# Antiparadox/Spartan-BN254

Measured on AMD Instinct MI355X. Metric: msm_points_per_s, higher is better.
Workload: dtype u32; 1 GPU; synthetic BN254 G1 MSM, 2^20 uniform Fr scalars x distinct bases per GPU, inputs resident in HBM; steps_in_flight=6

## Files before the change

spartan-bn254_amd/csrc/sort2_kernels.cuh:

```cuda
#pragma once
#include "msm_kernels.cuh"
#include <utility>

namespace sbn {

struct S2Geom {
  size_t n;
  int c, W, P;
  int lo_log;
  int K;
  size_t half, gap;
};

template <int C, int SW = 8> struct S2Shape {
  static constexpr int BITS = SW == 8 ? 254 : 127;
  static constexpr int W0 = (BITS + C - 1) / C;
  static constexpr int W = W0 + ((BITS - (W0 - 1) * C) > C - 1 ? 1 : 0);
};
typedef uint32_t s2_u32x8 __attribute__((ext_vector_type(8)));
template <int C, int w> __device__ __forceinline__ int s2_digit(const s2_u32x8 k, uint32_t& carry) {
  constexpr int bit = w * C, limb = bit >> 5, sh = bit & 31;
  uint64_t x = 0;
  if constexpr (limb < 8) x = k[limb];
  if constexpr (limb + 1 < 8) x |= (uint64_t)k[limb + 1] << 32;
  const uint32_t raw = (uint32_t)(x >> sh) & ((1u << C) - 1u);
  const uint32_t v = raw + carry;
  if (v >= (1u << (C - 1))) { carry = 1; return (int)v - (1 << C); }
  carry = 0;
  return (int)v;
}
template <int SW = 8> __device__ __forceinline__ s2_u32x8 s2_load_scalar(const uint32_t* __restrict__ scalars, size_t t) {
  const uint4* p = reinterpret_cast<const uint4*>(scalars + (size_t)SW * t);
  const uint4 a = p[0], b = SW == 8 ? p[1] : make_uint4(0u, 0u, 0u, 0u);
  s2_u32x8 k; k[0] = a.x; k[1] = a.y; k[2] = a.z; k[3] = a.w; k[4] = b.x; k[5] = b.y; k[6] = b.z; k[7] = b.w;
  return k;
}
__device__ __forceinline__ bool s2_is_canonical(const s2_u32x8 k) { uint32_t kk[8]; for (int i = 0; i < 8; i++) kk[i] = k[i]; return fe_is_canonical<FrP>(kk); }

extern __shared__ uint32_t s2_lds[];

template <int C, int... Ws>
__device__ __forceinline__ void s2_count_scalar(const s2_u32x8 kk, int P, int lo_log, std::integer_sequence<int, Ws...>) {
  uint32_t carry = 0;
  auto one = [&](auto wc) {
    constexpr int w = decltype(wc)::value;
    const int d = s2_digit<C, w>(kk, carry);
    if (d != 0) atomicAdd(&s2_lds[w * P + (((d < 0 ? -d : d) - 1) >> lo_log)], 1u);
  };
  (one(std::integral_constant<int, Ws>{}), ...);
}
template <int C, int SPT, int SW = 8>
__global__ void __launch_bounds__(1024) k_s2_count(const uint32_t* __restrict__ scalars, S2Geom g, uint32_t* __restrict__ cntA, uint32_t* __restrict__ bad) {
  constexpr int W = S2Shape<C, SW>::W; constexpr int CH = 1024 * SPT;
  const int k = blockIdx.x, P = g.P;
  for (int j = threadIdx.x; j < W * P; j += 1024) s2_lds[j] = 0;
  __syncthreads();
  for (int i = 0; i < SPT; i++) {
    const size_t t = (size_t)k * CH + (size_t)i * 1024 + threadIdx.x;
    if (t >= g.n) break;
    const s2_u32x8 kk = s2_load_scalar<SW>(scalars, t);
    if (SW == 8 && !s2_is_canonical(kk)) atomicAdd(bad, 1u);
    s2_count_scalar<C>(kk, P, g.lo_log, std::make_integer_sequence<int, W>{});
  }
  __syncthreads();
  for (int j = threadIdx.x; j < W * P; j += 1024) cntA[(size_t)j * g.K + k] = s2_lds[j];
}

__device__ __forceinline__ uint32_t s2_block_scan(uint32_t v, uint32_t* tmp , uint32_t* total) {
  const int lane = threadIdx.x & 63, wv = threadIdx.x >> 6, nw = (blockDim.x + 63) >> 6;
  uint32_t inc = v;
#pragma unroll
  for (int d = 1; d < 64; d <<= 1) { const uint32_t o = __shfl_up(inc, d); if (lane >= d) inc += o; }
  if (lane == 63) tmp[wv] = inc;
  __syncthreads();
  if (threadIdx.x == 0) { uint32_t run = 0; for (int i = 0; i < nw; i++) { const uint32_t x = tmp[i]; tmp[i] = run; run += x; } tmp[16] = run; }
  __syncthreads();
  const uint32_t r = inc - v + tmp[wv];
  *total = tmp[16];
  __syncthreads();
  return r;
}
__global__ void __launch_bounds__(256) k_s2_prefix_k(uint32_t* __restrict__ cntA, int K, uint32_t* __restrict__ part_cnt) {
  __shared__ uint32_t tmp[17];
  uint32_t* row = cntA + (size_t)blockIdx.x * K;
  const int per = (K + 255) / 256, b0 = threadIdx.x * per;
  uint32_t sum = 0;
  for (int i = 0; i < per; i++) if (b0 + i < K) sum += row[b0 + i];
  uint32_t total; uint32_t run = s2_block_scan(sum, tmp, &total);
  for (int i = 0; i < per; i++) if (b0 + i < K) { const uint32_t v = row[b0 + i]; row[b0 + i] = run; run += v; }
  if (threadIdx.x == 0) part_cnt[blockIdx.x] = total;
}
__global__ void __launch_bounds__(1024) k_s2_prefix_hi(const uint32_t* __restrict__ part_cnt, int W, int P, uint32_t* __restrict__ part_off, uint32_t* __restrict__ sc_off) {
  __shared__ uint32_t tmp[17];
  __shared__ uint32_t wstart[32];
  const int n = W * P, per = (n + 1023) / 1024, i0 = (int)threadIdx.x * per, i1 = (i0 + per < n) ? i0 + per : n;
  uint32_t sv = 0, sk = 0;
  for (int i = i0; i < i1; i++) { const uint32_t v = part_cnt[i]; sv += v; sk += (v + S2_SUB - 1) / S2_SUB; }
  uint32_t tv, tk;
  uint32_t rv = s2_block_scan(sv, tmp, &tv), rk = s2_block_scan(sk, tmp, &tk);
  for (int i = i0; i < i1; i++) { const uint32_t v = part_cnt[i]; part_off[i] = rv; sc_off[i] = rk; rv += v; rk += (v + S2_SUB - 1) / S2_SUB; }
  if (threadIdx.x == 0) sc_off[(size_t)n] = tk;
  __syncthreads();
  if ((int)threadIdx.x < W) wstart[threadIdx.x] = part_off[(size_t)threadIdx.x * P];
  __syncthreads();
  for (int i = i0; i < i1; i++) part_off[i] -= wstart[i / P];
}

__host__ __device__ inline size_t s2_scatter_lds_bytes(int P, int spt = S2_SPT) { return ((size_t)3 * P + 32) * 4 + (size_t)1024 * spt * 8; }
struct S2ScatterArgs {
  const uint32_t* cntA; const uint32_t* part_off; uint32_t* tmp_idx; uint16_t* tmp_lo;
  size_t n, half, gap; int P, K, k, lo_log;
};
template <int C, int w, int SPT>
__device__ __forceinline__ void s2_scatter_window(const s2_u32x8 (&kk)[SPT], uint32_t (&carry)[SPT], const S2ScatterArgs& a) {
  constexpr int CH = 1024 * SPT;
  const int P = a.P, tid = threadIdx.x;
  uint32_t* cnt = s2_lds; uint32_t* base = cnt + P; uint32_t* gdelta = base + P; uint32_t* tmp = gdelta + P;
  uint32_t* stage_idx = tmp + 32;
  uint16_t* stage_lo = reinterpret_cast<uint16_t*>(stage_idx + CH); uint16_t* stage_hi = stage_lo + CH;
  for (int j = tid; j < P; j += 1024) cnt[j] = 0;
  __syncthreads();
  int d[SPT]; uint32_t rank[SPT];
#pragma unroll
  for (int i = 0; i < SPT; i++) {
    const int dd = s2_digit<C, w>(kk[i], carry[i]);
    d[i] = dd; rank[i] = 0;
    if (dd != 0) rank[i] = atomicAdd(&cnt[((dd < 0 ? -dd : dd) - 1) >> a.lo_log], 1u);
  }
  __syncthreads();
  uint32_t total;
  {
    const uint32_t v = tid < P ? cnt[tid] : 0;
    const uint32_t r = s2_block_scan(v, tmp, &total);
    if (tid < P) { base[tid] = r; gdelta[tid] = a.part_off[(size_t)w * P + tid] + a.cntA[((size_t)w * P + tid) * a.K + a.k] - r; }
  }
  __syncthreads();
  const size_t t0 = (size_t)a.k * CH + tid;
#pragma unroll
  for (int i = 0; i < SPT; i++) {
    if (d[i] == 0) continue;
    const uint32_t b = (uint32_t)((d[i] < 0 ? -d[i] : d[i]) - 1), hi = b >> a.lo_log;
    const uint32_t pos = base[hi] + rank[i];
    size_t e = t0 + (size_t)i * 1024;
    if (a.gap && e >= a.half) e += a.gap;
    stage_idx[pos] = (uint32_t)e | (d[i] < 0 ? 0x80000000u : 0u);
    stage_lo[pos] = (uint16_t)(b & ((1u << a.lo_log) - 1u)); stage_hi[pos] = (uint16_t)hi;
  }
  __syncthreads();
  uint32_t* oi = a.tmp_idx + (size_t)w * a.n; uint16_t* ol = a.tmp_lo + (size_t)w * a.n;
  for (uint32_t j = tid; j < total; j += 1024) {
    const uint32_t pos = j + gdelta[stage_hi[j]];
    oi[pos] = stage_idx[j]; ol[pos] = stage_lo[j];
  }
  __syncthreads();
}
template <int C, int SPT, int... Ws>
__device__ __forceinline__ void s2_scatter_windows(const s2_u32x8 (&kk)[SPT], uint32_t (&carry)[SPT], const S2ScatterArgs& a, std::integer_sequence<int, Ws...>) {
  (s2_scatter_window<C, Ws, SPT>(kk, carry, a), ...);
}
template <int C, int SPT, int SW = 8>
__global__ void __launch_bounds__(1024) k_s2_scatter(const uint32_t* __restrict__ scalars, S2Geom g, const uint32_t* __restrict__ cntA ,
                                                     const uint32_t* __restrict__ part_off, uint32_t* __restrict__ tmp_idx, uint16_t* __restrict__ tmp_lo) {
  S2ScatterArgs a; a.cntA = cntA; a.part_off = part_off; a.tmp_idx = tmp_idx; a.tmp_lo = tmp_lo; a.n = g.n; a.P = g.P; a.K = g.K; a.k = blockIdx.x; a.lo_log = g.lo_log;
  a.half = g.half; a.gap = SW == 8 ? 0 : g.gap;
  s2_u32x8 kk[SPT]; uint32_t carry[SPT];
#pragma unroll
  for (int i = 0; i < SPT; i++) {
    const size_t t = (size_t)blockIdx.x * (1024 * SPT) + (size_t)i * 1024 + threadIdx.x;
    carry[i] = 0;
    kk[i] = t < g.n ? s2_load_scalar<SW>(scalars, t) : (s2_u32x8)(0u);
  }
  s2_scatter_windows<C, SPT>(kk, carry, a, std::make_integer_sequence<int, S2Shape<C, SW>::W>{});
}

__device__ __forceinline__ bool s2_decode(const S2Geom& g, const uint32_t* __restrict__ sc_off, int& q, uint32_t& sidx, uint32_t& k2) {
  const uint32_t Lid = blockIdx.x, xcd = Lid & 7u, slot = Lid >> 3;
  sidx = (slot >> 4) * 128u + xcd * 16u + (slot & 15u);
  const int WP = g.W * g.P;
  if (sidx >= sc_off[WP]) return false;
  int lo = 0, hi = WP;
  while (hi - lo > 1) { const int mid = (lo + hi) >> 1; if (sc_off[mid] <= sidx) lo = mid; else hi = mid; }
  q = lo; k2 = sidx - sc_off[q];
  return true;
}
__host__ __device__ inline uint32_t s2_level2_blocks(size_t max_subchunks) { return (uint32_t)(((max_subchunks + 127) / 128) * 128); }
__device__ __forceinline__ void s2_range(const S2Geom& g, const uint32_t* __restrict__ part_off, const uint32_t* __restrict__ part_cnt, int q, uint32_t k2, size_t& e0, size_t& e1) {
  const uint32_t start = part_off[q], cn = part_cnt[q];
  uint32_t a = k2 * S2_SUB, b = a + S2_SUB; if (a > cn) a = cn; if (b > cn) b = cn;
  const size_t w = (size_t)(q / g.P);
  e0 = w * g.n + start + a; e1 = w * g.n + start + b;
}
__global__ void __launch_bounds__(1024) k_s2_hist(const uint16_t* __restrict__ tmp_lo, S2Geom g, const uint32_t* __restrict__ part_off, const uint32_t* __restrict__ part_cnt, const uint32_t* __restrict__ sc_off, uint32_t* __restrict__ blockhist) {
  __shared__ uint32_t h[S2_LO_MAX];
  int q; uint32_t sidx, k2; if (!s2_decode(g, sc_off, q, sidx, k2)) return;
  const int LO = 1 << g.lo_log;
  for (int j = threadIdx.x; j < LO; j += 1024) h[j] = 0;
  __syncthreads();
  size_t e0, e1; s2_range(g, part_off, part_cnt, q, k2, e0, e1);
  for (size_t e = e0 + threadIdx.x; e < e1; e += 1024) atomicAdd(&h[tmp_lo[e]], 1u);
  __syncthreads();
  uint32_t* o = blockhist + (size_t)sidx * LO;
  for (int j = threadIdx.x; j < LO; j += 1024) o[j] = h[j];
}
__global__ void __launch_bounds__(1024) k_s2_prefix2(uint32_t* __restrict__ blockhist, S2Geom g, const uint32_t* __restrict__ part_off, const uint32_t* __restrict__ sc_off, uint32_t* __restrict__ hist, uint32_t* __restrict__ offs) {
  __shared__ uint32_t tmp[17];
  const int q = blockIdx.x, LO = 1 << g.lo_log, w = q / g.P, hi = q - w * g.P;
  const uint32_t s0 = sc_off[q], nk = sc_off[q + 1] - s0;
  const int j0 = 2 * threadIdx.x;
  uint32_t r0 = 0, r1 = 0;
  if (j0 < LO) {
    uint2* col = reinterpret_cast<uint2*>(blockhist + (size_t)s0 * LO + j0);
    for (uint32_t k = 0; k < nk; k++) { uint2* pq = col + (size_t)k * (LO / 2); const uint2 v = *pq; *pq = make_uint2(r0, r1); r0 += v.x; r1 += v.y; }
  }
  uint32_t total; const uint32_t r = s2_block_scan(r0 + r1, tmp, &total);
  if (j0 < LO) {
    const size_t b = ((size_t)w * g.P + hi) * LO + j0;
    hist[b] = r0; hist[b + 1] = r1;
    offs[b] = part_off[q] + r; offs[b + 1] = part_off[q] + r + r0;
  }
}
constexpr int S2_EPT = 8;
__host__ __device__ inline size_t s2_place_lds_bytes(int lo_log) { return ((size_t)3 * ((size_t)1 << lo_log) + 32) * 4 + (size_t)1024 * S2_EPT * 6; }
__global__ void __launch_bounds__(1024) k_s2_place(const uint16_t* __restrict__ tmp_lo, const uint32_t* __restrict__ tmp_idx, S2Geom g, const uint32_t* __restrict__ part_off, const uint32_t* __restrict__ part_cnt,
                                                   const uint32_t* __restrict__ sc_off, const uint32_t* __restrict__ blockhist ,
                                                   const uint32_t* __restrict__ offs, uint32_t* __restrict__ sorted, size_t estride) {
  constexpr uint32_t T = 1024 * S2_EPT;
  int q; uint32_t sidx, k2; if (!s2_decode(g, sc_off, q, sidx, k2)) return;
  const int LO = 1 << g.lo_log, tid = threadIdx.x;
  uint32_t* cnt = s2_lds; uint32_t* base = cnt + LO; uint32_t* cur = base + LO; uint32_t* tmp = cur + LO;
  uint32_t* stage_idx = tmp + 32; uint16_t* stage_lo = reinterpret_cast<uint16_t*>(stage_idx + T);
  const int w = q / g.P, hi = q - w * g.P;
  const size_t nb = (size_t)g.P << g.lo_log;
  const uint32_t* b0 = blockhist + (size_t)sidx * LO;
  const uint32_t* of = offs + (size_t)w * nb + ((size_t)hi << g.lo_log);
  for (int j = tid; j < LO; j += 1024) { cur[j] = of[j] + b0[j]; cnt[j] = 0; }
  __syncthreads();
  size_t e0, e1; s2_range(g, part_off, part_cnt, q, k2, e0, e1);
  uint32_t* out = sorted + (size_t)w * estride;
  for (size_t tile = e0; tile < e1; tile += T) {
    uint32_t lo[S2_EPT], idx[S2_EPT], rank[S2_EPT];
#pragma unroll
    for (int i = 0; i < S2_EPT; i++) {
      const size_t e = tile + (size_t)i * 1024 + tid;
      lo[i] = 0xffffffffu;
      if (e < e1) { lo[i] = tmp_lo[e]; idx[i] = tmp_idx[e]; rank[i] = atomicAdd(&cnt[lo[i]], 1u); }
    }
    __syncthreads();
    uint32_t total;
    {
      const int j0 = 2 * tid, j1 = 2 * tid + 1;
      const uint32_t v0 = j0 < LO ? cnt[j0] : 0, v1 = j1 < LO ? cnt[j1] : 0;
      const uint32_t r = s2_block_scan(v0 + v1, tmp, &total);
      if (j0 < LO) base[j0] = r;
      if (j1 < LO) base[j1] = r + v0;
    }
    __syncthreads();
#pragma unroll
    for (int i = 0; i < S2_EPT; i++) {
      if (lo[i] == 0xffffffffu) continue;
      const uint32_t pos = base[lo[i]] + rank[i];
      stage_idx[pos] = idx[i]; stage_lo[pos] = (uint16_t)lo[i];
    }
    __syncthreads();
    for (uint32_t j = tid; j < total; j += 1024) {
      const uint32_t l = stage_lo[j];
      out[cur[l] + (j - base[l])] = stage_idx[j];
    }
    __syncthreads();
    for (int j = tid; j < LO; j += 1024) { cur[j] += cnt[j]; cnt[j] = 0; }
    __syncthreads();
  }
}

}
```

spartan-bn254_amd/csrc/glv_kernels.cuh:

```cuda
#pragma once
#include "msm_kernels.cuh"

namespace sbn {

namespace glv {
constexpr uint64_t A[2] = {0x8211bbeb7d4f1128ull, 0x6f4d8248eeb859fcull};
constexpr uint64_t B = 0x89d3256894d213e3ull;
constexpr uint64_t C[2] = {0x0be4e1541221250bull, 0x6f4d8248eeb859fdull};
constexpr uint64_t G1[3] = {0x5398fd0300ff6565ull, 0x4ccef014a773d2d2ull, 0x2ull};
constexpr uint64_t G2[2] = {0xd91d232ec7e0b3d7ull, 0x2ull};
constexpr uint64_t R[4] = {0x43e1f593f0000001ull, 0x2833e84879b97091ull, 0xb85045b68181585dull, 0x30644e72e131a029ull};
constexpr uint32_t BETA[8] = {0x607cfd48u, 0xe4bd44e5u, 0xbb966e3du, 0xc28f069fu, 0xe0acccb0u, 0x5e6dd9e7u, 0xe131a029u, 0x30644e72u};
}

template <int NA, int NB>
__device__ __forceinline__ void glv_mul(const uint64_t (&a)[NA], const uint64_t (&b)[NB], uint64_t (&out)[NA + NB]) {
#pragma unroll
  for (int i = 0; i < NA + NB; i++) out[i] = 0;
#pragma unroll
  for (int i = 0; i < NA; i++) {
    uint64_t carry = 0;
#pragma unroll
    for (int j = 0; j < NB; j++) {
      const uint64_t lo = a[i] * b[j], hi = __umul64hi(a[i], b[j]);
      uint64_t s = out[i + j] + lo; uint64_t cy = s < lo ? 1 : 0;
      s += carry; cy += s < carry ? 1 : 0;
      out[i + j] = s; carry = hi + cy;
    }
    out[i + NB] = carry;
  }
}
template <int NB>
__device__ __forceinline__ void glv_mul_lo256(const uint64_t (&a)[4], const uint64_t (&b)[NB], uint64_t (&out)[4]) {
#pragma unroll
  for (int i = 0; i < 4; i++) out[i] = 0;
#pragma unroll
  for (int i = 0; i < 4; i++) {
    uint64_t carry = 0;
#pragma unroll
    for (int j = 0; j < NB && i + j < 4; j++) {
      const uint64_t lo = a[i] * b[j], hi = __umul64hi(a[i], b[j]);
      uint64_t s = out[i + j] + lo; uint64_t cy = s < lo ? 1 : 0;
      s += carry; cy += s < carry ? 1 : 0;
      out[i + j] = s; carry = hi + cy;
    }
    if (i + NB < 4) out[i + NB] = carry;
  }
}
__device__ __forceinline__ bool glv_diff_ge_r(const uint64_t (&x)[4], const uint64_t (&y)[4]) {
  uint64_t d[4], borrow = 0;
#pragma unroll
  for (int i = 0; i < 4; i++) { const uint64_t t = x[i] - y[i]; const uint64_t b1 = x[i] < y[i]; d[i] = t - borrow; borrow = b1 | (t < borrow); }
#pragma unroll
  for (int i = 3; i >= 0; i--) { if (d[i] != glv::R[i]) return d[i] > glv::R[i]; }
  return true;
}
__device__ __forceinline__ void u128_mul_lo(uint64_t a0, uint64_t a1, uint64_t b0, uint64_t b1, uint64_t& o0, uint64_t& o1) {
  o0 = a0 * b0; o1 = __umul64hi(a0, b0) + a0 * b1 + a1 * b0;
}
__device__ __forceinline__ void u128_add(uint64_t& x0, uint64_t& x1, uint64_t y0, uint64_t y1) { const uint64_t s = x0 + y0; x1 += y1 + (s < x0 ? 1 : 0); x0 = s; }
__device__ __forceinline__ void u128_sub(uint64_t& x0, uint64_t& x1, uint64_t y0, uint64_t y1) { const uint64_t b = x0 < y0 ? 1 : 0; x0 -= y0; x1 -= y1 + b; }

__device__ __forceinline__ void glv_split(const uint64_t (&k)[4], uint64_t (&k1)[2], uint64_t (&k2)[2]) {
  uint64_t p1[7], p2[6];
  glv_mul<4, 3>(k, glv::G1, p1);
  glv_mul<4, 2>(k, glv::G2, p2);
  uint64_t c1[2] = {p1[4], p1[5]}, c2[1] = {p2[4]};
  {
    uint64_t kc[4], cr[4];
    glv_mul_lo256<2>(k, glv::C, kc);
    const uint64_t c1v[4] = {c1[0], c1[1], 0, 0};
    glv_mul_lo256<4>(c1v, glv::R, cr);
    if (glv_diff_ge_r(kc, cr)) { if (++c1[0] == 0) ++c1[1]; }
  }
  {
    uint64_t kb[4], cr[4];
    const uint64_t bb[1] = {glv::B};
    glv_mul_lo256<1>(k, bb, kb);
    const uint64_t c2v[4] = {c2[0], 0, 0, 0};
    glv_mul_lo256<4>(c2v, glv::R, cr);
    if (glv_diff_ge_r(kb, cr)) ++c2[0];
  }
  uint64_t x0 = k[0], x1 = k[1], t0, t1;
  u128_mul_lo(c1[0], c1[1], glv::A[0], glv::A[1], t0, t1); u128_sub(x0, x1, t0, t1);
  u128_mul_lo(c2[0], 0, glv::B, 0, t0, t1); u128_sub(x0, x1, t0, t1);
  uint64_t y0, y1;
  u128_mul_lo(c1[0], c1[1], glv::B, 0, y0, y1);
  u128_mul_lo(c2[0], 0, glv::C[0], glv::C[1], t0, t1); u128_sub(y0, y1, t0, t1);
  if (y1 >> 63) { u128_add(x0, x1, glv::B, 0); u128_add(y0, y1, glv::C[0], glv::C[1]); }
  k1[0] = x0; k1[1] = x1; k2[0] = y0; k2[1] = y1;
}

__global__ void __launch_bounds__(256) k_glv_split(const uint32_t* __restrict__ scalars, size_t n, uint32_t* __restrict__ out, uint32_t* __restrict__ bad) {
  const size_t t = (size_t)blockIdx.x * blockDim.x + threadIdx.x;
  if (t >= n) return;
  const uint4 a = reinterpret_cast<const uint4*>(scalars + 8 * t)[0], b = reinterpret_cast<const uint4*>(scalars + 8 * t)[1];
  const uint32_t kk[8] = {a.x, a.y, a.z, a.w, b.x, b.y, b.z, b.w};
  uint64_t k1[2] = {0, 0}, k2[2] = {0, 0};
  if (!fe_is_canonical<FrP>(kk)) atomicAdd(bad, 1u);
  else {
    const uint64_t k[4] = {(uint64_t)a.x | ((uint64_t)a.y << 32), (uint64_t)a.z | ((uint64_t)a.w << 32), (uint64_t)b.x | ((uint64_t)b.y << 32), (uint64_t)b.z | ((uint64_t)b.w << 32)};
    glv_split(k, k1, k2);
  }
  uint4* o = reinterpret_cast<uint4*>(out);
  o[t] = make_uint4((uint32_t)k1[0], (uint32_t)(k1[0] >> 32), (uint32_t)k1[1], (uint32_t)(k1[1] >> 32));
  o[n + t] = make_uint4((uint32_t)k2[0], (uint32_t)(k2[0] >> 32), (uint32_t)k2[1], (uint32_t)(k2[1] >> 32));
}

__global__ void __launch_bounds__(256) k_glv_table(const uint32_t* __restrict__ pts, size_t npts, uint32_t* __restrict__ out) {
  const size_t j = (size_t)blockIdx.x * blockDim.x + threadIdx.x;
  if (j >= npts) return;
  const uint4* s = reinterpret_cast<const uint4*>(pts + 16 * j);
  uint4* d0 = reinterpret_cast<uint4*>(out + 16 * j);
  uint4* d1 = reinterpret_cast<uint4*>(out + 16 * (npts + j));
  const uint4 w0 = s[0], w1 = s[1], w2 = s[2], w3 = s[3];
  d0[0] = w0; d0[1] = w1; d0[2] = w2; d0[3] = w3;
  const Fq beta = fe_to_mont(fe_unpack<FqP>(glv::BETA));
  const Fq x = fe_load<FqP>(pts + 16 * j);
  fe_store<FqP>(out + 16 * (npts + j), fe_mul(x, beta));
  d1[2] = w2; d1[3] = w3;
}

}
```

Before: 788.2 million points/s.

## Cut barriers and prefetch in MSM sort scatter, hist and place kernels

The scatter kernel now double-buffers its per-window counters, packs the staging entries into uint2, prefetches the next window's global offset and drops several __syncthreads. Sub-chunk decode becomes a parallel search that also caches part_off and part_cnt in shared memory. The hist kernel reads tmp_lo eight entries at a time with uint4 loads. The place kernel loads both tiles of a sub-chunk up front, takes a fast path for sub-chunks of at most 1024 elements, and sets a launch-bounds occupancy hint. These changes target barrier and load-latency overhead in the bucket sort, at the cost of extra registers and tighter assumptions such as S2_SUB equal to two tiles.

```diff
diff --git a/spartan-bn254_amd/csrc/sort2_kernels.cuh b/spartan-bn254_amd/csrc/sort2_kernels.cuh
--- a/spartan-bn254_amd/csrc/sort2_kernels.cuh
+++ b/spartan-bn254_amd/csrc/sort2_kernels.cuh
@@ -66,7 +66,7 @@
   for (int j = threadIdx.x; j < W * P; j += 1024) cntA[(size_t)j * g.K + k] = s2_lds[j];
 }
 
-__device__ __forceinline__ uint32_t s2_block_scan(uint32_t v, uint32_t* tmp , uint32_t* total) {
+__device__ __forceinline__ uint32_t s2_block_scan_open(uint32_t v, uint32_t* tmp , uint32_t* total) {
   const int lane = threadIdx.x & 63, wv = threadIdx.x >> 6, nw = (blockDim.x + 63) >> 6;
   uint32_t inc = v;
 #pragma unroll
@@ -77,6 +77,10 @@
   __syncthreads();
   const uint32_t r = inc - v + tmp[wv];
   *total = tmp[16];
+  return r;
+}
+__device__ __forceinline__ uint32_t s2_block_scan(uint32_t v, uint32_t* tmp , uint32_t* total) {
+  const uint32_t r = s2_block_scan_open(v, tmp, total);
   __syncthreads();
   return r;
 }
@@ -111,15 +115,19 @@
   const uint32_t* cntA; const uint32_t* part_off; uint32_t* tmp_idx; uint16_t* tmp_lo;
   size_t n, half, gap; int P, K, k, lo_log;
 };
-template <int C, int w, int SPT>
-__device__ __forceinline__ void s2_scatter_window(const s2_u32x8 (&kk)[SPT], uint32_t (&carry)[SPT], const S2ScatterArgs& a) {
+__device__ __forceinline__ uint32_t s2_scatter_goff(const S2ScatterArgs& a, int w) {
+  const size_t j = (size_t)w * a.P + threadIdx.x;
+  return (int)threadIdx.x < a.P ? a.part_off[j] + a.cntA[j * a.K + a.k] : 0u;
+}
+template <int C, int w, int W, int SPT>
+__device__ __forceinline__ void s2_scatter_window(const s2_u32x8 (&kk)[SPT], uint32_t (&carry)[SPT], const S2ScatterArgs& a, uint32_t& gpre) {
   constexpr int CH = 1024 * SPT;
   const int P = a.P, tid = threadIdx.x;
-  uint32_t* cnt = s2_lds; uint32_t* base = cnt + P; uint32_t* gdelta = base + P; uint32_t* tmp = gdelta + P;
-  uint32_t* stage_idx = tmp + 32;
-  uint16_t* stage_lo = reinterpret_cast<uint16_t*>(stage_idx + CH); uint16_t* stage_hi = stage_lo + CH;
-  for (int j = tid; j < P; j += 1024) cnt[j] = 0;
-  __syncthreads();
+  uint2* stage = reinterpret_cast<uint2*>(s2_lds);
+  uint32_t* ctr = s2_lds + 2 * CH; uint32_t* gdelta = ctr + 2 * P; uint32_t* tmp = gdelta + P;
+  uint32_t* cnt = ctr + (w & 1) * P; uint32_t* other = ctr + ((w + 1) & 1) * P;
+  uint32_t gnext = 0;
+  if constexpr (w + 1 < W) gnext = s2_scatter_goff(a, w + 1);
   int d[SPT]; uint32_t rank[SPT];
 #pragma unroll
   for (int i = 0; i < SPT; i++) {
@@ -131,8 +139,9 @@
   uint32_t total;
   {
     const uint32_t v = tid < P ? cnt[tid] : 0;
-    const uint32_t r = s2_block_scan(v, tmp, &total);
-    if (tid < P) { base[tid] = r; gdelta[tid] = a.part_off[(size_t)w * P + tid] + a.cntA[((size_t)w * P + tid) * a.K + a.k] - r; }
+    if (tid < P) other[tid] = 0;
+    const uint32_t r = s2_block_scan_open(v, tmp, &total);
+    if (tid < P) { cnt[tid] = r; gdelta[tid] = gpre - r; }
   }
   __syncthreads();
   const size_t t0 = (size_t)a.k * CH + tid;
@@ -140,23 +149,23 @@
   for (int i = 0; i < SPT; i++) {
     if (d[i] == 0) continue;
     const uint32_t b = (uint32_t)((d[i] < 0 ? -d[i] : d[i]) - 1), hi = b >> a.lo_log;
-    const uint32_t pos = base[hi] + rank[i];
+    const uint32_t pos = cnt[hi] + rank[i];
     size_t e = t0 + (size_t)i * 1024;
     if (a.gap && e >= a.half) e += a.gap;
-    stage_idx[pos] = (uint32_t)e | (d[i] < 0 ? 0x80000000u : 0u);
-    stage_lo[pos] = (uint16_t)(b & ((1u << a.lo_log) - 1u)); stage_hi[pos] = (uint16_t)hi;
+    stage[pos] = make_uint2((uint32_t)e | (d[i] < 0 ? 0x80000000u : 0u), (b & ((1u << a.lo_log) - 1u)) | (hi << 16));
   }
   __syncthreads();
   uint32_t* oi = a.tmp_idx + (size_t)w * a.n; uint16_t* ol = a.tmp_lo + (size_t)w * a.n;
   for (uint32_t j = tid; j < total; j += 1024) {
-    const uint32_t pos = j + gdelta[stage_hi[j]];
-    oi[pos] = stage_idx[j]; ol[pos] = stage_lo[j];
-  }
-  __syncthreads();
+    const uint2 s = stage[j];
+    const uint32_t pos = j + gdelta[s.y >> 16];
+    oi[pos] = s.x; ol[pos] = (uint16_t)s.y;
+  }
+  gpre = gnext;
 }
 template <int C, int SPT, int... Ws>
-__device__ __forceinline__ void s2_scatter_windows(const s2_u32x8 (&kk)[SPT], uint32_t (&carry)[SPT], const S2ScatterArgs& a, std::integer_sequence<int, Ws...>) {
-  (s2_scatter_window<C, Ws, SPT>(kk, carry, a), ...);
+__device__ __forceinline__ void s2_scatter_windows(const s2_u32x8 (&kk)[SPT], uint32_t (&carry)[SPT], const S2ScatterArgs& a, uint32_t& gpre, std::integer_sequence<int, Ws...>) {
+  (s2_scatter_window<C, Ws, (int)sizeof...(Ws), SPT>(kk, carry, a, gpre), ...);
 }
 template <int C, int SPT, int SW = 8>
 __global__ void __launch_bounds__(1024) k_s2_scatter(const uint32_t* __restrict__ scalars, S2Geom g, const uint32_t* __restrict__ cntA ,
@@ -164,42 +173,62 @@
   S2ScatterArgs a; a.cntA = cntA; a.part_off = part_off; a.tmp_idx = tmp_idx; a.tmp_lo = tmp_lo; a.n = g.n; a.P = g.P; a.K = g.K; a.k = blockIdx.x; a.lo_log = g.lo_log;
   a.half = g.half; a.gap = SW == 8 ? 0 : g.gap;
   s2_u32x8 kk[SPT]; uint32_t carry[SPT];
+  uint32_t gpre = s2_scatter_goff(a, 0);
 #pragma unroll
   for (int i = 0; i < SPT; i++) {
     const size_t t = (size_t)blockIdx.x * (1024 * SPT) + (size_t)i * 1024 + threadIdx.x;
     carry[i] = 0;
     kk[i] = t < g.n ? s2_load_scalar<SW>(scalars, t) : (s2_u32x8)(0u);
   }
-  s2_scatter_windows<C, SPT>(kk, carry, a, std::make_integer_sequence<int, S2Shape<C, SW>::W>{});
-}
-
-__device__ __forceinline__ bool s2_decode(const S2Geom& g, const uint32_t* __restrict__ sc_off, int& q, uint32_t& sidx, uint32_t& k2) {
-  const uint32_t Lid = blockIdx.x, xcd = Lid & 7u, slot = Lid >> 3;
-  sidx = (slot >> 4) * 128u + xcd * 16u + (slot & 15u);
+  for (int j = threadIdx.x; j < 2 * g.P; j += 1024) s2_lds[2 * (1024 * SPT) + j] = 0;
+  __syncthreads();
+  s2_scatter_windows<C, SPT>(kk, carry, a, gpre, std::make_integer_sequence<int, S2Shape<C, SW>::W>{});
+}
+
+struct S2Sub { int q; uint32_t sidx, k2, start, cn; };
+__device__ __forceinline__ bool s2_decode(const S2Geom& g, const uint32_t* __restrict__ sc_off, const uint32_t* __restrict__ part_off, const uint32_t* __restrict__ part_cnt, uint32_t* sh, S2Sub& s) {
+  const uint32_t Lid = blockIdx.x, xcd = Lid & 7u, slot = Lid >> 3, sidx = (slot >> 4) * 128u + xcd * 16u + (slot & 15u);
   const int WP = g.W * g.P;
-  if (sidx >= sc_off[WP]) return false;
-  int lo = 0, hi = WP;
-  while (hi - lo > 1) { const int mid = (lo + hi) >> 1; if (sc_off[mid] <= sidx) lo = mid; else hi = mid; }
-  q = lo; k2 = sidx - sc_off[q];
+  const uint32_t nsc = sc_off[WP];
+  for (int j = threadIdx.x; j < WP; j += blockDim.x) {
+    const uint32_t a = sc_off[j], b = sc_off[j + 1];
+    if (a <= sidx && sidx < b) { sh[0] = (uint32_t)j; sh[1] = sidx - a; sh[2] = part_off[j]; sh[3] = part_cnt[j]; }
+  }
+  if (sidx >= nsc) return false;
+  __syncthreads();
+  s.sidx = sidx; s.q = (int)sh[0]; s.k2 = sh[1]; s.start = sh[2]; s.cn = sh[3];
   return true;
 }
 __host__ __device__ inline uint32_t s2_level2_blocks(size_t max_subchunks) { return (uint32_t)(((max_subchunks + 127) / 128) * 128); }
-__device__ __forceinline__ void s2_range(const S2Geom& g, const uint32_t* __restrict__ part_off, const uint32_t* __restrict__ part_cnt, int q, uint32_t k2, size_t& e0, size_t& e1) {
-  const uint32_t start = part_off[q], cn = part_cnt[q];
-  uint32_t a = k2 * S2_SUB, b = a + S2_SUB; if (a > cn) a = cn; if (b > cn) b = cn;
-  const size_t w = (size_t)(q / g.P);
-  e0 = w * g.n + start + a; e1 = w * g.n + start + b;
+__device__ __forceinline__ void s2_range(const S2Geom& g, const S2Sub& s, size_t& e0, size_t& e1) {
+  uint32_t a = s.k2 * S2_SUB, b = a + S2_SUB; if (a > s.cn) a = s.cn; if (b > s.cn) b = s.cn;
+  const size_t w = (size_t)(s.q / g.P);
+  e0 = w * g.n + s.start + a; e1 = w * g.n + s.start + b;
 }
 __global__ void __launch_bounds__(1024) k_s2_hist(const uint16_t* __restrict__ tmp_lo, S2Geom g, const uint32_t* __restrict__ part_off, const uint32_t* __restrict__ part_cnt, const uint32_t* __restrict__ sc_off, uint32_t* __restrict__ blockhist) {
   __shared__ uint32_t h[S2_LO_MAX];
-  int q; uint32_t sidx, k2; if (!s2_decode(g, sc_off, q, sidx, k2)) return;
+  __shared__ uint32_t dec[4];
   const int LO = 1 << g.lo_log;
   for (int j = threadIdx.x; j < LO; j += 1024) h[j] = 0;
-  __syncthreads();
-  size_t e0, e1; s2_range(g, part_off, part_cnt, q, k2, e0, e1);
-  for (size_t e = e0 + threadIdx.x; e < e1; e += 1024) atomicAdd(&h[tmp_lo[e]], 1u);
-  __syncthreads();
-  uint32_t* o = blockhist + (size_t)sidx * LO;
+  S2Sub s; if (!s2_decode(g, sc_off, part_off, part_cnt, dec, s)) return;
+  size_t e0, e1; s2_range(g, s, e0, e1);
+  const size_t a0 = ((e0 + 7) & ~(size_t)7) < e1 ? ((e0 + 7) & ~(size_t)7) : e1, a1 = a0 + ((e1 - a0) & ~(size_t)7);
+  if (e0 + threadIdx.x < a0) atomicAdd(&h[tmp_lo[e0 + threadIdx.x]], 1u);
+  if (a1 + threadIdx.x < e1) atomicAdd(&h[tmp_lo[a1 + threadIdx.x]], 1u);
+  const uint4* v = reinterpret_cast<const uint4*>(tmp_lo + a0);
+  const uint32_t ng = (uint32_t)((a1 - a0) >> 3);
+  auto add8 = [&](const uint4 x) {
+    atomicAdd(&h[x.x & 0xffffu], 1u); atomicAdd(&h[x.x >> 16], 1u); atomicAdd(&h[x.y & 0xffffu], 1u); atomicAdd(&h[x.y >> 16], 1u);
+    atomicAdd(&h[x.z & 0xffffu], 1u); atomicAdd(&h[x.z >> 16], 1u); atomicAdd(&h[x.w & 0xffffu], 1u); atomicAdd(&h[x.w >> 16], 1u);
+  };
+  for (uint32_t i = threadIdx.x; i < ng; i += 2048) {
+    const bool two = i + 1024 < ng;
+    const uint4 x = v[i], y = two ? v[i + 1024] : make_uint4(0u, 0u, 0u, 0u);
+    add8(x);
+    if (two) add8(y);
+  }
+  __syncthreads();
+  uint32_t* o = blockhist + (size_t)s.sidx * LO;
   for (int j = threadIdx.x; j < LO; j += 1024) o[j] = h[j];
 }
 __global__ void __launch_bounds__(1024) k_s2_prefix2(uint32_t* __restrict__ blockhist, S2Geom g, const uint32_t* __restrict__ part_off, const uint32_t* __restrict__ sc_off, uint32_t* __restrict__ hist, uint32_t* __restrict__ offs) {
@@ -221,51 +250,80 @@
 }
 constexpr int S2_EPT = 8;
 __host__ __device__ inline size_t s2_place_lds_bytes(int lo_log) { return ((size_t)3 * ((size_t)1 << lo_log) + 32) * 4 + (size_t)1024 * S2_EPT * 6; }
-__global__ void __launch_bounds__(1024) k_s2_place(const uint16_t* __restrict__ tmp_lo, const uint32_t* __restrict__ tmp_idx, S2Geom g, const uint32_t* __restrict__ part_off, const uint32_t* __restrict__ part_cnt,
+__global__ void __launch_bounds__(1024, 8) k_s2_place(const uint16_t* __restrict__ tmp_lo, const uint32_t* __restrict__ tmp_idx, S2Geom g, const uint32_t* __restrict__ part_off, const uint32_t* __restrict__ part_cnt,
                                                    const uint32_t* __restrict__ sc_off, const uint32_t* __restrict__ blockhist ,
                                                    const uint32_t* __restrict__ offs, uint32_t* __restrict__ sorted, size_t estride) {
   constexpr uint32_t T = 1024 * S2_EPT;
-  int q; uint32_t sidx, k2; if (!s2_decode(g, sc_off, q, sidx, k2)) return;
+  static_assert(S2_SUB == 2 * T, "a sub-chunk is two tiles: both are loaded before the first is sorted");
   const int LO = 1 << g.lo_log, tid = threadIdx.x;
   uint32_t* cnt = s2_lds; uint32_t* base = cnt + LO; uint32_t* cur = base + LO; uint32_t* tmp = cur + LO;
   uint32_t* stage_idx = tmp + 32; uint16_t* stage_lo = reinterpret_cast<uint16_t*>(stage_idx + T);
-  const int w = q / g.P, hi = q - w * g.P;
+  S2Sub s; if (!s2_decode(g, sc_off, part_off, part_cnt, tmp + 20, s)) return;
+  const int w = s.q / g.P, hi = s.q - w * g.P;
   const size_t nb = (size_t)g.P << g.lo_log;
-  const uint32_t* b0 = blockhist + (size_t)sidx * LO;
+  const uint32_t* b0 = blockhist + (size_t)s.sidx * LO;
   const uint32_t* of = offs + (size_t)w * nb + ((size_t)hi << g.lo_log);
-  for (int j = tid; j < LO; j += 1024) { cur[j] = of[j] + b0[j]; cnt[j] = 0; }
-  __syncthreads();
-  size_t e0, e1; s2_range(g, part_off, part_cnt, q, k2, e0, e1);
+  size_t e0, e1; s2_range(g, s, e0, e1);
   uint32_t* out = sorted + (size_t)w * estride;
-  for (size_t tile = e0; tile < e1; tile += T) {
-    uint32_t lo[S2_EPT], idx[S2_EPT], rank[S2_EPT];
+  const uint32_t m = (uint32_t)(e1 - e0);
+  if (m <= 1024) {
+    uint32_t l = 0, ix = 0, dst = 0;
+    const bool have = (uint32_t)tid < m;
+    if (have) { l = tmp_lo[e0 + tid]; ix = tmp_idx[e0 + tid]; dst = of[l] + b0[l]; cnt[l] = 0; }
+    __syncthreads();
+    if (have) out[dst + atomicAdd(&cnt[l], 1u)] = ix;
+    return;
+  }
+  uint32_t c0[2];
+#pragma unroll
+  for (int i = 0; i < 2; i++) { const int j = tid + 1024 * i; c0[i] = j < LO ? of[j] + b0[j] : 0u; }
+  uint32_t lo[2][S2_EPT], idx[2][S2_EPT];
+#pragma unroll
+  for (int t = 0; t < 2; t++) {
 #pragma unroll
     for (int i = 0; i < S2_EPT; i++) {
-      const size_t e = tile + (size_t)i * 1024 + tid;
-      lo[i] = 0xffffffffu;
-      if (e < e1) { lo[i] = tmp_lo[e]; idx[i] = tmp_idx[e]; rank[i] = atomicAdd(&cnt[lo[i]], 1u); }
+      const size_t e = e0 + (size_t)t * T + (size_t)i * 1024 + tid;
+      lo[t][i] = e < e1 ? (uint32_t)tmp_lo[e] : 0xffffffffu;
+    }
+#pragma unroll
+    for (int i = 0; i < S2_EPT; i++) {
+      const size_t e = e0 + (size_t)t * T + (size_t)i * 1024 + tid;
+      idx[t][i] = e < e1 ? tmp_idx[e] : 0u;
+    }
+  }
+#pragma unroll
+  for (int i = 0; i < 2; i++) { const int j = tid + 1024 * i; if (j < LO) { cur[j] = c0[i]; cnt[j] = 0; } }
+  __syncthreads();
+#pragma unroll
+  for (int t = 0; t < 2; t++) {
+    uint32_t rank[S2_EPT];
+#pragma unroll
+    for (int i = 0; i < S2_EPT; i++) {
+      rank[i] = 0;
+      if (lo[t][i] != 0xffffffffu) rank[i] = atomicAdd(&cnt[lo[t][i]], 1u);
     }
     __syncthreads();
     uint32_t total;
     {
       const int j0 = 2 * tid, j1 = 2 * tid + 1;
       const uint32_t v0 = j0 < LO ? cnt[j0] : 0, v1 = j1 < LO ? cnt[j1] : 0;
-      const uint32_t r = s2_block_scan(v0 + v1, tmp, &total);
+      const uint32_t r = s2_block_scan_open(v0 + v1, tmp, &total);
       if (j0 < LO) base[j0] = r;
       if (j1 < LO) base[j1] = r + v0;
     }
     __syncthreads();
 #pragma unroll
     for (int i = 0; i < S2_EPT; i++) {
-      if (lo[i] == 0xffffffffu) continue;
-      const uint32_t pos = base[lo[i]] + rank[i];
-      stage_idx[pos] = idx[i]; stage_lo[pos] = (uint16_t)lo[i];
+      if (lo[t][i] == 0xffffffffu) continue;
+      const uint32_t pos = base[lo[t][i]] + rank[i];
+      stage_idx[pos] = idx[t][i]; stage_lo[pos] = (uint16_t)lo[t][i];
     }
     __syncthreads();
     for (uint32_t j = tid; j < total; j += 1024) {
       const uint32_t l = stage_lo[j];
       out[cur[l] + (j - base[l])] = stage_idx[j];
     }
+    if (t == 1 || m <= T) break;
     __syncthreads();
     for (int j = tid; j < LO; j += 1024) { cur[j] += cnt[j]; cnt[j] = 0; }
     __syncthreads();
```

Result: no change. 787.5 million points/s (-0.1%).

## Rewrite GLV split in 29-bit limbs and streamline scatter window scan

Applied to the files above, without the earlier changes.

The GLV scalar decomposition is reimplemented with 29-bit limb column accumulation on 32-bit multiplies, computing rounding corrections as branchless masks instead of 64-bit carry chains with data-dependent branches. The scatter kernel replaces the generic block scan with a wave-shuffle scan, packs the lo and hi bucket indices into one 32-bit LDS word, moves index math to 32 bits, and drops a barrier per window by clearing the counts inside the scan. This reduces 64-bit integer work and LDS and synchronisation overhead, but adds correctness risk in the new limb arithmetic and in the 32-bit index assumptions.

```diff
diff --git a/spartan-bn254_amd/csrc/glv_kernels.cuh b/spartan-bn254_amd/csrc/glv_kernels.cuh
--- a/spartan-bn254_amd/csrc/glv_kernels.cuh
+++ b/spartan-bn254_amd/csrc/glv_kernels.cuh
@@ -13,95 +13,134 @@
 constexpr uint32_t BETA[8] = {0x607cfd48u, 0xe4bd44e5u, 0xbb966e3du, 0xc28f069fu, 0xe0acccb0u, 0x5e6dd9e7u, 0xe131a029u, 0x30644e72u};
 }
 
+namespace glv {
+constexpr uint32_t LM = (1u << 29) - 1u;
+template <int NW> constexpr uint32_t limb29(const uint64_t (&w)[NW], int i) {
+  const int bit = 29 * i, q = bit >> 6, s = bit & 63;
+  uint64_t x = q < NW ? w[q] >> s : 0;
+  if (s > 35 && q + 1 < NW) x |= w[q + 1] << (64 - s);
+  return (uint32_t)x & LM;
+}
+constexpr uint64_t BW[1] = {B};
+constexpr uint64_t GS1[3] = {0x731fa0601fecaca2ull, 0x99de0294ee7a5a4aull, 0x49ull};
+constexpr uint64_t GS2[2] = {0x23a465d8fc167aedull, 0x5bull};
+constexpr uint32_t A29[5] = {limb29(A, 0), limb29(A, 1), limb29(A, 2), limb29(A, 3), limb29(A, 4)};
+constexpr uint32_t B29[3] = {limb29(BW, 0), limb29(BW, 1), limb29(BW, 2)};
+constexpr uint32_t C29[5] = {limb29(C, 0), limb29(C, 1), limb29(C, 2), limb29(C, 3), limb29(C, 4)};
+constexpr uint32_t GS1_29[5] = {limb29(GS1, 0), limb29(GS1, 1), limb29(GS1, 2), limb29(GS1, 3), limb29(GS1, 4)};
+constexpr uint32_t GS2_29[3] = {limb29(GS2, 0), limb29(GS2, 1), limb29(GS2, 2)};
+constexpr uint32_t R29[9] = {limb29(R, 0), limb29(R, 1), limb29(R, 2), limb29(R, 3), limb29(R, 4), limb29(R, 5), limb29(R, 6), limb29(R, 7), limb29(R, 8)};
+}
+
+#if defined(__HIP_DEVICE_COMPILE__)
+#define SBN_GLV_PIN(x) asm volatile("" ::"v"(x))
+__device__ __forceinline__ uint32_t glv_word(uint32_t x) { uint32_t r; asm("v_mov_b32 %0, %1" : "=v"(r) : "v"(x)); return r; }
+#else
+#define SBN_GLV_PIN(x) ((void)0)
+__device__ __forceinline__ uint32_t glv_word(uint32_t x) { return x; }
+#endif
 template <int NA, int NB>
-__device__ __forceinline__ void glv_mul(const uint64_t (&a)[NA], const uint64_t (&b)[NB], uint64_t (&out)[NA + NB]) {
+__device__ __forceinline__ void glv_col(uint64_t& acc, const uint32_t (&a)[NA], const uint32_t (&b)[NB], int col) {
 #pragma unroll
-  for (int i = 0; i < NA + NB; i++) out[i] = 0;
+  for (int i = 0; i < NA; i++) { const int j = col - i; if (j >= 0 && j < NB) { acc += (uint64_t)a[i] * (uint64_t)b[j]; SBN_GLV_PIN(acc); } }
+}
+template <int LO, int HI, int FIRST = 0, int NA, int NB>
+__device__ __forceinline__ void glv_cols(const uint32_t (&a)[NA], const uint32_t (&b)[NB], uint32_t (&out)[HI - LO + 1]) {
+  uint64_t acc = 0;
 #pragma unroll
-  for (int i = 0; i < NA; i++) {
-    uint64_t carry = 0;
-#pragma unroll
-    for (int j = 0; j < NB; j++) {
-      const uint64_t lo = a[i] * b[j], hi = __umul64hi(a[i], b[j]);
-      uint64_t s = out[i + j] + lo; uint64_t cy = s < lo ? 1 : 0;
-      s += carry; cy += s < carry ? 1 : 0;
-      out[i + j] = s; carry = hi + cy;
-    }
-    out[i + NB] = carry;
+  for (int col = FIRST; col <= HI; col++) {
+    glv_col(acc, a, b, col);
+    if (col >= LO) out[col - LO] = col < HI ? (uint32_t)acc & glv::LM : (uint32_t)acc;
+    acc >>= 29; SBN_GLV_PIN(acc);
   }
 }
-template <int NB>
-__device__ __forceinline__ void glv_mul_lo256(const uint64_t (&a)[4], const uint64_t (&b)[NB], uint64_t (&out)[4]) {
+template <int N, int NM, int NA, int NB, int NC, int ND>
+__device__ __forceinline__ void glv_minus_cols2(const uint32_t (&m)[NM], const uint32_t (&a)[NA], const uint32_t (&b)[NB], const uint32_t (&c)[NC], const uint32_t (&d)[ND], uint32_t (&out)[N]) {
+  uint64_t acc = 0;
+  int32_t cy = 0;
 #pragma unroll
-  for (int i = 0; i < 4; i++) out[i] = 0;
-#pragma unroll
-  for (int i = 0; i < 4; i++) {
-    uint64_t carry = 0;
-#pragma unroll
-    for (int j = 0; j < NB && i + j < 4; j++) {
-      const uint64_t lo = a[i] * b[j], hi = __umul64hi(a[i], b[j]);
-      uint64_t s = out[i + j] + lo; uint64_t cy = s < lo ? 1 : 0;
-      s += carry; cy += s < carry ? 1 : 0;
-      out[i + j] = s; carry = hi + cy;
-    }
-    if (i + NB < 4) out[i + NB] = carry;
+  for (int col = 0; col < N; col++) {
+    glv_col(acc, a, b, col); glv_col(acc, c, d, col);
+    const int32_t t = (int32_t)(m[col] - ((uint32_t)acc & glv::LM)) + cy;
+    out[col] = (uint32_t)t & glv::LM; cy = t >> 29;
+    acc >>= 29; SBN_GLV_PIN(acc);
   }
 }
-__device__ __forceinline__ bool glv_diff_ge_r(const uint64_t (&x)[4], const uint64_t (&y)[4]) {
-  uint64_t d[4], borrow = 0;
+template <int N, int NA, int NB, int NC, int ND>
+__device__ __forceinline__ void glv_diff_cols(const uint32_t (&a)[NA], const uint32_t (&b)[NB], const uint32_t (&c)[NC], const uint32_t (&d)[ND], uint32_t (&out)[N]) {
+  uint64_t p = 0, q = 0;
+  int32_t cy = 0;
 #pragma unroll
-  for (int i = 0; i < 4; i++) { const uint64_t t = x[i] - y[i]; const uint64_t b1 = x[i] < y[i]; d[i] = t - borrow; borrow = b1 | (t < borrow); }
+  for (int col = 0; col < N; col++) {
+    glv_col(p, a, b, col); glv_col(q, c, d, col);
+    const int32_t t = (int32_t)(((uint32_t)p & glv::LM) - ((uint32_t)q & glv::LM)) + cy;
+    out[col] = (uint32_t)t & glv::LM; cy = t >> 29;
+    p >>= 29; SBN_GLV_PIN(p); q >>= 29; SBN_GLV_PIN(q);
+  }
+}
+template <bool PLUS, int NA, int NB>
+__device__ __forceinline__ uint32_t glv_rem_ge_r(const uint32_t (&x)[5], const uint32_t (&a)[NA], const uint32_t (&y)[5], const uint32_t (&b)[NB], uint32_t neg) {
+  uint64_t p = 0, q = 0;
+  int32_t d = 0;
 #pragma unroll
-  for (int i = 3; i >= 0; i--) { if (d[i] != glv::R[i]) return d[i] > glv::R[i]; }
-  return true;
+  for (int col = 0; col < 9; col++) {
+    glv_col(p, x, a, col);
+    if (PLUS) glv_col(p, y, b, col); else glv_col(q, y, b, col);
+    int32_t t = (int32_t)((uint32_t)p & glv::LM) - (int32_t)glv::R29[col];
+    if (!PLUS) t -= (int32_t)((uint32_t)q & glv::LM);
+    if (col >= 5 && col - 5 < NB) t += PLUS ? -(int32_t)(neg & b[col - 5]) : (int32_t)(neg & b[col - 5]);
+    d = (d >> 29) + t;
+    p >>= 29; SBN_GLV_PIN(p);
+    if (!PLUS) { q >>= 29; SBN_GLV_PIN(q); }
+  }
+  return 0u - ((((uint32_t)d >> 28) & 1u) ^ 1u);
 }
-__device__ __forceinline__ void u128_mul_lo(uint64_t a0, uint64_t a1, uint64_t b0, uint64_t b1, uint64_t& o0, uint64_t& o1) {
-  o0 = a0 * b0; o1 = __umul64hi(a0, b0) + a0 * b1 + a1 * b0;
+__device__ __forceinline__ unsigned __int128 glv_u128(const uint32_t (&v)[5]) {
+  typedef unsigned __int128 u128;
+  return (u128)v[0] | ((u128)v[1] << 29) | ((u128)v[2] << 58) | ((u128)v[3] << 87) | ((u128)v[4] << 116);
 }
-__device__ __forceinline__ void u128_add(uint64_t& x0, uint64_t& x1, uint64_t y0, uint64_t y1) { const uint64_t s = x0 + y0; x1 += y1 + (s < x0 ? 1 : 0); x0 = s; }
-__device__ __forceinline__ void u128_sub(uint64_t& x0, uint64_t& x1, uint64_t y0, uint64_t y1) { const uint64_t b = x0 < y0 ? 1 : 0; x0 -= y0; x1 -= y1 + b; }
+__device__ __forceinline__ unsigned __int128 glv_masked(uint64_t lo, uint64_t hi, uint32_t m) {
+  const uint64_t mm = ((uint64_t)m << 32) | m;
+  return ((unsigned __int128)(hi & mm) << 64) | (lo & mm);
+}
 
 __device__ __forceinline__ void glv_split(const uint64_t (&k)[4], uint64_t (&k1)[2], uint64_t (&k2)[2]) {
-  uint64_t p1[7], p2[6];
-  glv_mul<4, 3>(k, glv::G1, p1);
-  glv_mul<4, 2>(k, glv::G2, p2);
-  uint64_t c1[2] = {p1[4], p1[5]}, c2[1] = {p2[4]};
-  {
-    uint64_t kc[4], cr[4];
-    glv_mul_lo256<2>(k, glv::C, kc);
-    const uint64_t c1v[4] = {c1[0], c1[1], 0, 0};
-    glv_mul_lo256<4>(c1v, glv::R, cr);
-    if (glv_diff_ge_r(kc, cr)) { if (++c1[0] == 0) ++c1[1]; }
-  }
-  {
-    uint64_t kb[4], cr[4];
-    const uint64_t bb[1] = {glv::B};
-    glv_mul_lo256<1>(k, bb, kb);
-    const uint64_t c2v[4] = {c2[0], 0, 0, 0};
-    glv_mul_lo256<4>(c2v, glv::R, cr);
-    if (glv_diff_ge_r(kb, cr)) ++c2[0];
-  }
-  uint64_t x0 = k[0], x1 = k[1], t0, t1;
-  u128_mul_lo(c1[0], c1[1], glv::A[0], glv::A[1], t0, t1); u128_sub(x0, x1, t0, t1);
-  u128_mul_lo(c2[0], 0, glv::B, 0, t0, t1); u128_sub(x0, x1, t0, t1);
-  uint64_t y0, y1;
-  u128_mul_lo(c1[0], c1[1], glv::B, 0, y0, y1);
-  u128_mul_lo(c2[0], 0, glv::C[0], glv::C[1], t0, t1); u128_sub(y0, y1, t0, t1);
-  if (y1 >> 63) { u128_add(x0, x1, glv::B, 0); u128_add(y0, y1, glv::C[0], glv::C[1]); }
-  k1[0] = x0; k1[1] = x1; k2[0] = y0; k2[1] = y1;
+  typedef unsigned __int128 u128;
+  uint32_t kl[9];
+#pragma unroll
+  for (int i = 0; i < 9; i++) kl[i] = glv::limb29(k, i);
+  uint32_t c1[5], c2[3];
+  glv_cols<9, 13, 7>(kl, glv::GS1_29, c1); c1[4] = glv_word(c1[4]);
+  glv_cols<9, 11, 7>(kl, glv::GS2_29, c2); c2[2] = glv_word(c2[2]);
+  uint32_t x[5], y[5];
+  glv_minus_cols2(kl, c1, glv::A29, c2, glv::B29, x);
+  glv_diff_cols(c1, glv::B29, c2, glv::C29, y);
+  const uint32_t neg = 0u - (y[4] >> 28);
+  const uint32_t e1 = glv_rem_ge_r<false>(x, glv::C29, y, glv::B29, neg);
+  const uint32_t e2 = glv_rem_ge_r<true>(x, glv::B29, y, glv::A29, neg);
+  u128 X = glv_u128(x), Y = glv_u128(y);
+  X -= glv_masked(glv::A[0], glv::A[1], e1); X -= glv_masked(glv::B, 0, e2);
+  Y += glv_masked(glv::B, 0, e1); Y -= glv_masked(glv::C[0], glv::C[1], e2);
+  const uint32_t e3 = 0u - (uint32_t)(Y >> 127);
+  X += glv_masked(glv::B, 0, e3); Y += glv_masked(glv::C[0], glv::C[1], e3);
+  k1[0] = (uint64_t)X; k1[1] = (uint64_t)(X >> 64); k2[0] = (uint64_t)Y; k2[1] = (uint64_t)(Y >> 64);
 }
 
-__global__ void __launch_bounds__(256) k_glv_split(const uint32_t* __restrict__ scalars, size_t n, uint32_t* __restrict__ out, uint32_t* __restrict__ bad) {
+__device__ __forceinline__ bool glv_is_canonical(const uint64_t (&k)[4]) {
+  typedef unsigned __int128 u128;
+  const u128 hi = ((u128)k[3] << 64) | k[2], lo = ((u128)k[1] << 64) | k[0];
+  const u128 rhi = ((u128)glv::R[3] << 64) | glv::R[2], rlo = ((u128)glv::R[1] << 64) | glv::R[0];
+  return hi < rhi || (hi == rhi && lo < rlo);
+}
+
+__global__ void __launch_bounds__(256, 8) k_glv_split(const uint32_t* __restrict__ scalars, size_t n, uint32_t* __restrict__ out, uint32_t* __restrict__ bad) {
   const size_t t = (size_t)blockIdx.x * blockDim.x + threadIdx.x;
   if (t >= n) return;
   const uint4 a = reinterpret_cast<const uint4*>(scalars + 8 * t)[0], b = reinterpret_cast<const uint4*>(scalars + 8 * t)[1];
-  const uint32_t kk[8] = {a.x, a.y, a.z, a.w, b.x, b.y, b.z, b.w};
+  const uint64_t k[4] = {(uint64_t)a.x | ((uint64_t)a.y << 32), (uint64_t)a.z | ((uint64_t)a.w << 32), (uint64_t)b.x | ((uint64_t)b.y << 32), (uint64_t)b.z | ((uint64_t)b.w << 32)};
   uint64_t k1[2] = {0, 0}, k2[2] = {0, 0};
-  if (!fe_is_canonical<FrP>(kk)) atomicAdd(bad, 1u);
-  else {
-    const uint64_t k[4] = {(uint64_t)a.x | ((uint64_t)a.y << 32), (uint64_t)a.z | ((uint64_t)a.w << 32), (uint64_t)b.x | ((uint64_t)b.y << 32), (uint64_t)b.z | ((uint64_t)b.w << 32)};
-    glv_split(k, k1, k2);
-  }
+  if (!glv_is_canonical(k)) atomicAdd(bad, 1u);
+  else glv_split(k, k1, k2);
   uint4* o = reinterpret_cast<uint4*>(out);
   o[t] = make_uint4((uint32_t)k1[0], (uint32_t)(k1[0] >> 32), (uint32_t)k1[1], (uint32_t)(k1[1] >> 32));
   o[n + t] = make_uint4((uint32_t)k2[0], (uint32_t)(k2[0] >> 32), (uint32_t)k2[1], (uint32_t)(k2[1] >> 32));
diff --git a/spartan-bn254_amd/csrc/sort2_kernels.cuh b/spartan-bn254_amd/csrc/sort2_kernels.cuh
--- a/spartan-bn254_amd/csrc/sort2_kernels.cuh
+++ b/spartan-bn254_amd/csrc/sort2_kernels.cuh
@@ -109,17 +109,16 @@
 __host__ __device__ inline size_t s2_scatter_lds_bytes(int P, int spt = S2_SPT) { return ((size_t)3 * P + 32) * 4 + (size_t)1024 * spt * 8; }
 struct S2ScatterArgs {
   const uint32_t* cntA; const uint32_t* part_off; uint32_t* tmp_idx; uint16_t* tmp_lo;
-  size_t n, half, gap; int P, K, k, lo_log;
+  size_t n; uint32_t half, gap; int P, K, k, lo_log;
 };
 template <int C, int w, int SPT>
 __device__ __forceinline__ void s2_scatter_window(const s2_u32x8 (&kk)[SPT], uint32_t (&carry)[SPT], const S2ScatterArgs& a) {
   constexpr int CH = 1024 * SPT;
-  const int P = a.P, tid = threadIdx.x;
+  const int P = a.P, tid = threadIdx.x, lane = tid & 63, wv = tid >> 6;
   uint32_t* cnt = s2_lds; uint32_t* base = cnt + P; uint32_t* gdelta = base + P; uint32_t* tmp = gdelta + P;
-  uint32_t* stage_idx = tmp + 32;
-  uint16_t* stage_lo = reinterpret_cast<uint16_t*>(stage_idx + CH); uint16_t* stage_hi = stage_lo + CH;
-  for (int j = tid; j < P; j += 1024) cnt[j] = 0;
-  __syncthreads();
+  uint32_t* stage_idx = tmp + 32; uint32_t* stage_lohi = stage_idx + CH;
+  uint32_t gstart = 0;
+  if (tid < P) gstart = a.part_off[(size_t)w * P + tid] + a.cntA[((size_t)w * P + tid) * a.K + a.k];
   int d[SPT]; uint32_t rank[SPT];
 #pragma unroll
   for (int i = 0; i < SPT; i++) {
@@ -128,31 +127,40 @@
     if (dd != 0) rank[i] = atomicAdd(&cnt[((dd < 0 ? -dd : dd) - 1) >> a.lo_log], 1u);
   }
   __syncthreads();
-  uint32_t total;
-  {
-    const uint32_t v = tid < P ? cnt[tid] : 0;
-    const uint32_t r = s2_block_scan(v, tmp, &total);
-    if (tid < P) { base[tid] = r; gdelta[tid] = a.part_off[(size_t)w * P + tid] + a.cntA[((size_t)w * P + tid) * a.K + a.k] - r; }
-  }
-  __syncthreads();
-  const size_t t0 = (size_t)a.k * CH + tid;
+  uint32_t v = 0;
+  if (tid < P) { v = cnt[tid]; cnt[tid] = 0; }
+  uint32_t inc = v;
+#pragma unroll
+  for (int s = 1; s < 64; s <<= 1) { const uint32_t o = __shfl_up(inc, s); if (lane >= s) inc += o; }
+  if (lane == 63) tmp[wv] = inc;
+  __syncthreads();
+  uint32_t ws = lane < 16 ? tmp[lane] : 0;
+#pragma unroll
+  for (int s = 1; s < 16; s <<= 1) { const uint32_t o = __shfl_up(ws, s); if (lane >= s) ws += o; }
+  const uint32_t total = __shfl(ws, 15), before = __shfl(ws, wv > 0 ? wv - 1 : 0);
+  if (tid < P) { const uint32_t r = inc - v + (wv > 0 ? before : 0u); base[tid] = r; gdelta[tid] = gstart - r; }
+  __syncthreads();
+  const uint32_t t0 = (uint32_t)a.k * (uint32_t)CH + (uint32_t)tid;
 #pragma unroll
   for (int i = 0; i < SPT; i++) {
     if (d[i] == 0) continue;
     const uint32_t b = (uint32_t)((d[i] < 0 ? -d[i] : d[i]) - 1), hi = b >> a.lo_log;
     const uint32_t pos = base[hi] + rank[i];
-    size_t e = t0 + (size_t)i * 1024;
-    if (a.gap && e >= a.half) e += a.gap;
-    stage_idx[pos] = (uint32_t)e | (d[i] < 0 ? 0x80000000u : 0u);
-    stage_lo[pos] = (uint16_t)(b & ((1u << a.lo_log) - 1u)); stage_hi[pos] = (uint16_t)hi;
+    uint32_t e = t0 + (uint32_t)i * 1024u;
+    e += e >= a.half ? a.gap : 0u;
+    stage_idx[pos] = e | (d[i] < 0 ? 0x80000000u : 0u);
+    stage_lohi[pos] = (b & ((1u << a.lo_log) - 1u)) | (hi << 16);
   }
   __syncthreads();
   uint32_t* oi = a.tmp_idx + (size_t)w * a.n; uint16_t* ol = a.tmp_lo + (size_t)w * a.n;
-  for (uint32_t j = tid; j < total; j += 1024) {
-    const uint32_t pos = j + gdelta[stage_hi[j]];
-    oi[pos] = stage_idx[j]; ol[pos] = stage_lo[j];
-  }
-  __syncthreads();
+#pragma unroll
+  for (int i = 0; i < SPT; i++) {
+    const uint32_t j = (uint32_t)tid + (uint32_t)i * 1024u;
+    if (j < total) {
+      const uint32_t lh = stage_lohi[j], pos = j + gdelta[lh >> 16];
+      oi[pos] = stage_idx[j]; ol[pos] = (uint16_t)lh;
+    }
+  }
 }
 template <int C, int SPT, int... Ws>
 __device__ __forceinline__ void s2_scatter_windows(const s2_u32x8 (&kk)[SPT], uint32_t (&carry)[SPT], const S2ScatterArgs& a, std::integer_sequence<int, Ws...>) {
@@ -162,7 +170,7 @@
 __global__ void __launch_bounds__(1024) k_s2_scatter(const uint32_t* __restrict__ scalars, S2Geom g, const uint32_t* __restrict__ cntA ,
                                                      const uint32_t* __restrict__ part_off, uint32_t* __restrict__ tmp_idx, uint16_t* __restrict__ tmp_lo) {
   S2ScatterArgs a; a.cntA = cntA; a.part_off = part_off; a.tmp_idx = tmp_idx; a.tmp_lo = tmp_lo; a.n = g.n; a.P = g.P; a.K = g.K; a.k = blockIdx.x; a.lo_log = g.lo_log;
-  a.half = g.half; a.gap = SW == 8 ? 0 : g.gap;
+  a.half = SW == 8 ? 0xffffffffu : (uint32_t)g.half; a.gap = SW == 8 ? 0u : (uint32_t)g.gap;
   s2_u32x8 kk[SPT]; uint32_t carry[SPT];
 #pragma unroll
   for (int i = 0; i < SPT; i++) {
@@ -170,6 +178,8 @@
     carry[i] = 0;
     kk[i] = t < g.n ? s2_load_scalar<SW>(scalars, t) : (s2_u32x8)(0u);
   }
+  for (int j = threadIdx.x; j < g.P; j += 1024) s2_lds[j] = 0;
+  __syncthreads();
   s2_scatter_windows<C, SPT>(kk, carry, a, std::make_integer_sequence<int, S2Shape<C, SW>::W>{});
 }
 
```

After: 779.8 million points/s before, 786.5 million points/s after (median of 6 runs). About the same (+0.9%).
